# Nuralamsiddik16/Ultrafnd_git

Hardware: AMD Instinct MI355X
Metric: train-step samples/sec (FakeSV batch, seq128+224^2) (higher is better)
Workload: dtype bf16

## Files before the change

include/ultrafnd_hip.h:

```cpp
#ifndef ULTRAFND_HIP_H
#define ULTRAFND_HIP_H

#include <stddef.h>
#include <stdint.h>

#ifdef __cplusplus
extern "C" {
#endif

#define UFND_OK 0
#define UFND_ERR_INVALID 1
#define UFND_ERR_LAUNCH 2

#define UFND_ABI_VERSION 6

const char* ufnd_last_error(void);
int ufnd_abi_version(void);

typedef struct ufnd_step_state {
  uint64_t step;
  uint64_t seed;
  float lr;
  float weight_decay;
  float beta1, beta2, eps;
// ... 144 lines not shown
  float a_eps, r_eps;
  int width;
  int tile_cfg;
  const void* residual_bf16;
  int ldrb;
  float* guard;
} ufnd_gemm_ln;
#define UFND_FOLD_GUARD_SLOTS 1024
int ufnd_gemm_bf16_ln(const void* A, const void* W, const float* bias, const float* residual, void* out_bf16,
                      float* out_f32, int M, int N, int K, int lda, int ldw, int ldr, int ldo, int ldf, int act,
                      const ufnd_gemm_ln* ln, void* stream);
int ufnd_gemm_bf16_stat_parts(int M, int N, int K);

int ufnd_ln_fold_guard(const float* stats, int M, int parts, int width, float eps, float* guard, void* stream);

int ufnd_gemm_bf16_tile_count(void);
int ufnd_gemm_bf16_tile_info(int tile_cfg, int* bm, int* bn, int* ln_aware);

int ufnd_layernorm(const float* x, int ldx, const float* gamma, const float* beta, void* out_bf16, float* out_f32,
                   int M, int H, float eps, void* stream);

int ufnd_attention_bf16(const void* qkv, const int32_t* key_mask, void* ctx, int B, int L, int heads,
                        void* stream);

int ufnd_qkv_attention_bf16(const void* X, const void* Wqkv, const float* bqkv, const int32_t* key_mask, void* ctx, int B, int L,
                            int heads, int ldx, int ldw, const ufnd_gemm_ln* ln, void* stream);

int ufnd_text_pack(const int32_t* mask, int B, int L, int32_t* cu_seqlens, int32_t* row_src, void* stream);
int ufnd_text_pack_bins(const int32_t* mask, int B, int L, int32_t* cu_seqlens, int32_t* row_src, int32_t* bins, int32_t* nbins,
                        void* stream);
int ufnd_bert_embed_live(const int64_t* ids, const int32_t* row_src, const int* m_live, const float* word, const float* pos,
                         const float* type0, const float* gamma, const float* beta, void* x_bf16, float* x_f32, int capacity, int L,
                         int H, int vocab, float eps, void* stream);
int ufnd_gemm_bf16_live(const void* A, const void* W, const float* bias, const float* residual, void* out_bf16, float* out_f32,
                        int M, int N, int K, int lda, int ldw, int ldr, int ldo, int ldf, int act, int tile_cfg, const int* m_live,
                        void* stream);
int ufnd_gemm_bf16_ln_live(const void* A, const void* W, const float* bias, const float* residual, void* out_bf16, float* out_f32,
                           int M, int N, int K, int lda, int ldw, int ldr, int ldo, int ldf, int act, const ufnd_gemm_ln* ln,
                           const int* m_live, void* stream);
int ufnd_qkv_attention_bf16_packed(const void* X, const void* Wqkv, const float* bqkv, const int32_t* key_mask, const int32_t* cu_seqlens,
                                   void* ctx, int B, int L, int heads, int ldx, int ldw, const ufnd_gemm_ln* ln, void* stream);
int ufnd_qkv_attention_bf16_bins(const void* X, const void* Wqkv, const float* bqkv, const int32_t* key_mask, const int32_t* cu_seqlens,
                                 const int32_t* bins, const int32_t* nbins, void* ctx, int B, int L, int heads, int ldx, int ldw,
                                 const ufnd_gemm_ln* ln, void* stream);
int ufnd_attention_bf16_varlen_masked(const void* qkv, const int32_t* cu_seqlens, const int32_t* key_mask, void* ctx, int B, int max_len,
                                      int heads, void* stream);

int ufnd_qkv_attention_bf16_vit(const void* X, const void* Wqkv, const float* bqkv, void* ctx, int N, int T, int heads, int ldx, int ldw,
                                const ufnd_gemm_ln* ln, void* stream);
int ufnd_layernorm_live(const float* x, int ldx, const float* gamma, const float* beta, void* out_bf16, float* out_f32, int capacity,
                        int H, float eps, const int* m_live, void* stream);
int ufnd_masked_meanpool_l2_live(const float* hidden, const int32_t* mask, const int32_t* cu_seqlens, float* out, int B, int L, int H,
                                 void* stream);

int ufnd_bert_embed(const int64_t* ids, const float* word, const float* pos, const float* type0, const float* gamma,
                    const float* beta, void* x_bf16, float* x_f32, int B, int L, int H, int vocab, float eps,
                    void* stream);

int ufnd_masked_meanpool_l2(const float* hidden, const int32_t* mask, float* out, int B, int L, int H,
                            void* stream);

int ufnd_field_mean_l2(const float* parts, const int32_t* valid, float* out, int N, int M, int D, void* stream);

int ufnd_vit_patchify(const float* frames, void* patches_bf16, int N, int image, int patch, void* stream);

int ufnd_vit_assemble(const float* patch_emb, const float* cls, const float* pos, const float* gamma,
                      const float* beta, float* x_f32, void* x_bf16, float* stats, int N, int P, int H, float eps,
                      void* stream);

int ufnd_l2norm_frames(const float* e, float* out, int B, int F, int D, void* stream);

#define UFND_GATHER_MAX_ITEMS 8
typedef struct ufnd_gather_item {
  const void* src;
  void* dst;
  int row_bytes;
  int64_t src_rows;
} ufnd_gather_item;
int ufnd_gather_rows(const int64_t* idx, int B, const ufnd_gather_item* items, int n_items, void* stream);

int ufnd_temporal_weight_ld(int in_dim);
size_t ufnd_temporal_workspace_floats(int B, int in_dim, int hidden);
int ufnd_temporal_align(const float* text, const float* visual, const float* w0, const float* b0, const float* w3,
                        const float* b3, float* workspace, float* out, int B, int in_dim, int vis_dim, int hidden,
                        int out_dim, float dropout_p, const ufnd_step_state* state, void* stream);

typedef struct ufnd_tcn_layer {
  const float *w, *b;
  const float *gamma, *beta;
  float *running_mean, *running_var;
} ufnd_tcn_layer;
int ufnd_tcn_weight_ld(int in_ch, int kernel);
size_t ufnd_tcn_workspace_floats(int B, int T, int in_ch, int hid, int kernel);
int ufnd_tcn_forward(const float* text_seq, int text_dim, const float* vis_seq, int vis_dim, int B, int T,
                     const ufnd_tcn_layer* layers, int n_layers, int kernel, int hid, const float* head_w,
                     const float* head_b, int out_dim, int train, float dropout_p, float momentum, float eps,
                     const ufnd_step_state* state, float* workspace, float* out, void* stream);


int ufnd_ocr_adjacency(const int32_t* offsets, const int32_t* tokens, int N, double thresh, float* adj, int ld, void* stream);

typedef struct ufnd_gcn_params {
  const float* w1;
  const float* b1;
  const float* w2;
  const float* b2;
// ... 175 lines not shown
```

ultrafnd_git_amd/_lib.py:

```python
from __future__ import annotations

import ctypes as C
from pathlib import Path
from typing import Optional

import torch

_PKG = Path(__file__).resolve().parent
LIB_PATH = _PKG / "libultrafnd_hip.so"


class UltrafndHipError(RuntimeError):
    pass


class StepState(C.Structure):
    _fields_ = [("step", C.c_uint64), ("seed", C.c_uint64), ("lr", C.c_float), ("weight_decay", C.c_float),
                ("beta1", C.c_float), ("beta2", C.c_float), ("eps", C.c_float), ("max_norm", C.c_float),
                ("grad_scale", C.c_float), ("loss", C.c_float), ("grad_norm", C.c_float), ("clip_coef", C.c_float),
                ("bc1", C.c_float), ("bc2_sqrt", C.c_float), ("micro", C.c_uint32), ("reserved", C.c_float * 2)]


class Dims(C.Structure):
    _fields_ = [("hidden", C.c_int), ("text_dim", C.c_int), ("audio_dim", C.c_int), ("visual_dim", C.c_int),
# ... 101 lines not shown
                                             I, P, P, P, I]
    lib.ufnd_classifier_backward_ex.argtypes = [C.POINTER(Dims), C.POINTER(ClfParams), C.POINTER(ClfParams), I, I, P, P, P,
                                                I, P, P, P, I, I]
    lib.ufnd_classifier_backward_ex.restype = I
    lib.ufnd_head_factor_floats.argtypes = [C.POINTER(Dims), I]
    lib.ufnd_head_factor_floats.restype = S
    lib.ufnd_head_pack_factors.argtypes = [C.POINTER(Dims), P, P, P, P, P, I, P, P, P, P]
    lib.ufnd_head_pack_factors.restype = I
    lib.ufnd_head_linear_grads_from_factors.argtypes = [C.POINTER(Dims), C.POINTER(FusionParams), C.POINTER(ClfParams), P, S, I, I, P]
    lib.ufnd_head_linear_grads_from_factors.restype = I
    lib.ufnd_head_forward_loss.argtypes = [C.POINTER(Dims), C.POINTER(FusionParams), C.POINTER(ClfParams), C.POINTER(HeadIO), I, I, P, P]
    lib.ufnd_head_forward_loss.restype = I
    lib.ufnd_head_backward.argtypes = [C.POINTER(Dims), C.POINTER(FusionParams), C.POINTER(FusionParams), C.POINTER(ClfParams), C.POINTER(ClfParams),
                                       C.POINTER(HeadIO), I, I, P, P, P, I, I]
    lib.ufnd_head_backward.restype = I
    lib.ufnd_softmax_ce.argtypes = [P, P, I, P, P, P, P]
    lib.ufnd_softmax_ce_weighted.argtypes = [P, P, I, C.c_float, C.c_float, C.c_float, P, P, P, P]
    lib.ufnd_softmax_ce_weighted.restype = I
    lib.ufnd_grad_norm.argtypes = [P, S, P, P, P]
    lib.ufnd_adamw_step.argtypes = [P, P, P, P, S, P, P]
    lib.ufnd_step_advance.argtypes = [P, P]
    lib.ufnd_clip_adamw_step.argtypes = [P, P, P, P, S, P, P, P]
    lib.ufnd_clip_adamw_step.restype = I
    lib.ufnd_grad_accumulate.argtypes = [P, P, S, I, P, P]
    lib.ufnd_grad_accumulate.restype = I
    for name in ("ufnd_fusion_forward", "ufnd_fusion_backward", "ufnd_classifier_forward", "ufnd_classifier_backward",
                 "ufnd_softmax_ce", "ufnd_grad_norm", "ufnd_adamw_step", "ufnd_step_advance"):
        getattr(lib, name).restype = I
    _declare_encoders(lib)


def _declare_encoders(lib: C.CDLL) -> None:
    P, I, S, F = C.c_void_p, C.c_int, C.c_size_t, C.c_float
    sigs = {
        "ufnd_cast_bf16": [P, P, S, P],
        "ufnd_gemm_bf16": [P] * 6 + [I] * 9 + [P],
        "ufnd_gemm_bf16_ex": [P] * 6 + [I] * 10 + [P],
        "ufnd_layernorm": [P, I, P, P, P, P, I, I, F, P],
        "ufnd_attention_bf16": [P, P, P, I, I, I, P],
        "ufnd_qkv_attention_bf16": [P, P, P, P, P, I, I, I, I, I, C.POINTER(GemmLn), P],
        "ufnd_bert_embed": [P] * 8 + [I, I, I, I, F, P],
        "ufnd_masked_meanpool_l2": [P, P, P, I, I, I, P],
        "ufnd_text_pack": [P, I, I, P, P, P],
        "ufnd_text_pack_bins": [P, I, I, P, P, P, P, P],
        "ufnd_bert_embed_live": [P] * 10 + [I, I, I, I, F, P],
        "ufnd_gemm_bf16_live": [P] * 6 + [I] * 10 + [P, P],
        "ufnd_gemm_bf16_ln_live": [P] * 6 + [I] * 9 + [C.POINTER(GemmLn), P, P],
        "ufnd_qkv_attention_bf16_packed": [P, P, P, P, P, P, I, I, I, I, I, C.POINTER(GemmLn), P],
        "ufnd_qkv_attention_bf16_bins": [P] * 8 + [I, I, I, I, I, C.POINTER(GemmLn), P],
        "ufnd_qkv_attention_bf16_vit": [P, P, P, P, I, I, I, I, I, C.POINTER(GemmLn), P],
        "ufnd_attention_bf16_varlen_masked": [P, P, P, P, I, I, I, P],
        "ufnd_layernorm_live": [P, I, P, P, P, P, I, I, F, P, P],
        "ufnd_masked_meanpool_l2_live": [P, P, P, P, I, I, I, P],
        "ufnd_vit_patchify": [P, P, I, I, I, P],
        "ufnd_vit_assemble": [P] * 8 + [I, I, I, F, P],
        "ufnd_gemm_bf16_ln": [P] * 6 + [I] * 9 + [C.POINTER(GemmLn), P],
        "ufnd_gemm_bf16_stat_parts": [I, I, I],
        "ufnd_ln_fold_guard": [P, I, I, I, F, P, P],
        "ufnd_gemm_bf16_tile_count": [],
        "ufnd_gemm_bf16_tile_info": [I, C.POINTER(I), C.POINTER(I), C.POINTER(I)],
        "ufnd_stream_create_cu_mask": [C.POINTER(C.c_uint32), I, C.POINTER(P)],
        "ufnd_stream_destroy": [P],
        "ufnd_device_cu_count": [],
        "ufnd_l2norm_frames": [P, P, I, I, I, P],
        "ufnd_field_mean_l2": [P, P, P, I, I, I, P],
        "ufnd_temporal_align": [P] * 8 + [I] * 5 + [F, P, P],
    }
    sigs.update({
        "ufnd_gemm_bf16_dgrad": [P] * 6 + [I] * 10 + [P],
        "ufnd_gemm_bf16_wgrad": [P, P, P, I, I, I, I, I, I, P, I, P],
        "ufnd_transpose_bf16": [P, I, I, I, I, P, I, I, P, P, I, P],
        "ufnd_linear_wgrad": [P, I, P, I, I, I, I, P, P, P, P, I, P, P, C.POINTER(PartialsJob), I, P],
        "ufnd_refresh_operands": [P, I, I, P],
        "ufnd_layernorm_bwd_blocks": [I],
        "ufnd_row_partials_finish": [C.POINTER(PartialsJob), I, P],
        "ufnd_attention_bf16_lse": [P, P, P, P, I, I, I, P],
        "ufnd_attention_bf16_bwd": [P, P, P, P, P, P, P, I, I, I, P],
        "ufnd_layernorm_bwd": [P, I, P, P, I, P, I, P, P, I, P, P, P, I, I, I, F, P],
        "ufnd_masked_meanpool_l2_bwd": [P, P, P, P, I, I, I, P],
        "ufnd_l2norm_frames_bwd": [P, P, P, I, I, I, P],
        "ufnd_bert_embed_bwd": [P, P, P, P, P, I, I, I, I, I, I, P],
        "ufnd_vit_assemble_bwd": [P, P, P, P, I, I, I, P],
        "ufnd_act_bf16": [P, P, S, I, P],
        "ufnd_attention_bf16_lse_dropout": [P, P, P, P, I, I, I, C.POINTER(Dropout), P],
        "ufnd_attention_bf16_bwd_dropout": [P, P, P, P, P, P, P, I, I, I, C.POINTER(Dropout), P],
        "ufnd_dropout_residual_layernorm": [P, I, P, I, P, P, P, P, P, I, I, F, C.POINTER(Dropout), P],
        "ufnd_layernorm_dropout": [P, I, P, P, P, P, I, I, F, C.POINTER(Dropout), P],
        "ufnd_layernorm_bwd_dropout": [P, I, P, P, I, P, I, P, P, I, P, P, P, I, I, I, F, C.POINTER(Dropout), I, P],
    })
    sigs.update({
        "ufnd_wave_normalize": [P, P, P, P, I, I, P],
        "ufnd_w2v2_conv0": [P] * 8 + [I, I, I, F, P],
        "ufnd_conv1d_rows_bf16": [P] * 5 + [I] * 8 + [P],
        "ufnd_w2v2_pos_pack": [P, P, P, I, I, P],
        "ufnd_w2v2_pos_add": [P, P, P, P, I, I, P],
        "ufnd_w2v2_frames": [P, P, P, I, I, P],
        "ufnd_masked_meanpool": [P, P, P, I, I, I, P],
        "ufnd_linear_f32": [P, P, P, P, I, I, I, P],
    })
    for name, argtypes in sigs.items():
        fn = getattr(lib, name)
        fn.argtypes = argtypes
        fn.restype = I
    for name, argtypes in (("ufnd_gemm_bf16_wgrad_workspace_floats", [I, I, I]), ("ufnd_transpose_colsum_workspace_floats", [I, I]),
                           ("ufnd_attention_bwd_workspace_floats", [I, I, I]), ("ufnd_layernorm_bwd_workspace_floats", [I, I])):
        fn = getattr(lib, name)
# ... 107 lines not shown
```

ultrafnd_git_amd/csrc/encoders.hip:

```cpp
#include "common.hpp"

namespace {

__device__ __forceinline__ f32x4 ld4(const float* p) { return *reinterpret_cast<const f32x4*>(p); }

template <int NI>
__device__ __forceinline__ void ln_row(f32x4 (&v)[NI], int H, float eps, const float* gamma, const float* beta, int lane) {
  float s = 0.0f;
#pragma unroll
  for (int i = 0; i < NI; ++i) s += v[i][0] + v[i][1] + v[i][2] + v[i][3];
  const float mean = wave_sum(s) / (float)H;
  float q = 0.0f;
#pragma unroll
  for (int i = 0; i < NI; ++i)
#pragma unroll
    for (int k = 0; k < 4; ++k) {
      const float d = v[i][k] - mean;
      q += d * d;
    }
  const float rstd = rsqrtf(wave_sum(q) / (float)H + eps);
#pragma unroll
  for (int i = 0; i < NI; ++i) {
    const int col = 4 * lane + 256 * i;
    const f32x4 gm = ld4(gamma + col), bt = ld4(beta + col);
// ... 81 lines not shown
  long long id = ids[src];
  id = id < 0 ? 0 : (id >= vocab ? vocab - 1 : id);
  int l = src % L;
  l = l < 0 ? 0 : (l >= L ? L - 1 : l);
  f32x4 v[NI];
#pragma unroll
  for (int i = 0; i < NI; ++i) {
    const int col = 4 * lane + 256 * i;
    v[i] = ld4(word + (size_t)id * H + col) + ld4(pos + (size_t)l * H + col) + ld4(type0 + col);
  }
  if (gamma) ln_row<NI>(v, H, eps, gamma, beta, lane);
  store_row<NI>(v, ob, of, row, H, lane);
}

template <bool PACKED>
__global__ __launch_bounds__(256) void meanpool_kernel(const float* hidden, const int32_t* mask, float* out, int L, int H, const int32_t* cu) {
  __shared__ f32x4 part[4][64];
  __shared__ float cnts[4];
  const int b = blockIdx.y, col = blockIdx.x * 256 + 4 * (threadIdx.x & 63), grp = threadIdx.x >> 6, lane = threadIdx.x & 63;
  f32x4 acc = {0.f, 0.f, 0.f, 0.f};
  float cnt = 0.0f;
  const size_t r0 = PACKED ? (size_t)cu[b] : (size_t)b * L;
  const int n = PACKED ? cu[b + 1] - cu[b] : L;
  for (int l0 = grp; l0 < n; l0 += 32) {
    int mk[8];
    f32x4 x[8];
#pragma unroll
    for (int u = 0; u < 8; ++u) {
      const int l = l0 + 4 * u;
      mk[u] = l < n ? mask[(size_t)b * L + l] : 0;
    }
#pragma unroll
    for (int u = 0; u < 8; ++u) {
      const int l = l0 + 4 * u < n ? l0 + 4 * u : n - 1;
      x[u] = ld4(hidden + (r0 + l) * H + col);
    }
#pragma unroll
    for (int u = 0; u < 8; ++u) {
      if (mk[u] != 0) {
        acc += x[u];
        cnt += 1.0f;
      }
    }
  }
  part[grp][lane] = acc;
  if (lane == 0) cnts[grp] = cnt;
  __syncthreads();
  if (grp == 0) {
    const f32x4 s = (part[0][lane] + part[1][lane]) + (part[2][lane] + part[3][lane]);
    const float denom = fmaxf((cnts[0] + cnts[1]) + (cnts[2] + cnts[3]), 1e-6f);
    *reinterpret_cast<f32x4*>(out + (size_t)b * H + col) = s / denom;
  }
}
constexpr int PACK_THREADS = 1024, PACK_MAX_B = 16384;
__global__ __launch_bounds__(PACK_THREADS) void text_pack_kernel(const int32_t* mask, int B, int L, int32_t* cu, int32_t* row_src,
                                                                 int32_t* bins, int32_t* nbins) {
  __shared__ int lens[PACK_MAX_B];
  __shared__ int wsum[PACK_THREADS / 64];
  __shared__ long long csum[PACK_THREADS / 64];
  __shared__ int total;
  const int tid = threadIdx.x, wave = tid >> 6, lane = tid & 63;
  for (int b = wave; b < B; b += PACK_THREADS / 64) {
    int last = 0;
    for (int l = lane; l < L; l += 64) last = mask[(size_t)b * L + l] != 0 ? l + 1 : last;
#pragma unroll
    for (int o = 32; o >= 1; o >>= 1) last = max(last, __shfl_xor(last, o, 64));
    if (lane == 0) lens[b] = last;
  }
  __syncthreads();
  const int per = (B + PACK_THREADS - 1) / PACK_THREADS, b0 = tid * per, b1 = min(b0 + per, B);
  int own = 0;
  for (int b = b0; b < b1; ++b) own += lens[b];
  int inc = own;
#pragma unroll
  for (int o = 1; o < 64; o <<= 1) {
    const int y = __shfl_up(inc, o, 64);
    if (lane >= o) inc += y;
  }
  if (lane == 63) wsum[wave] = inc;
  __syncthreads();
  int base = 0;
  for (int w = 0; w < wave; ++w) base += wsum[w];
  int run = base + inc - own;
  for (int b = b0; b < b1; ++b) {
    const int n = lens[b];
    lens[b] = run;
    cu[b] = run;
    run += n;
  }
  if (tid == PACK_THREADS - 1) {
    cu[B] = run;
    total = run;
  }
  __syncthreads();
  for (int b = wave; b < B; b += PACK_THREADS / 64) {
    const int r0 = lens[b], n = (b + 1 < B ? lens[b + 1] : total) - r0;
    for (int l = lane; l < n; l += 64) row_src[r0 + l] = b * L + l;
  }
  if (!bins) return;
  auto nrows = [&](int b) { return (b + 1 < B ? lens[b + 1] : total) - lens[b]; };
  long long cown = 0;
  for (int b = b0; b < b1; ++b) {
    const int c = (nrows(b) + 31) >> 5;
    if (c > 0) cown += 1ll << (16 * (c - 1));
  }
  long long cinc = cown;
// ... 268 lines not shown
  UFND_REQUIRE(mask && cu_seqlens && row_src, "text_pack: null argument");
  UFND_REQUIRE(B >= 1 && B <= PACK_MAX_B && L >= 1 && (long long)B * L < (1ll << 31), "text_pack: B=%d L=%d (B <= %d)", B, L, PACK_MAX_B);
  hipLaunchKernelGGL(text_pack_kernel, dim3(1), dim3(PACK_THREADS), 0, (hipStream_t)stream_, mask, B, L, cu_seqlens, row_src,
                     (int32_t*)nullptr, (int32_t*)nullptr);
  UFND_CHECK_LAUNCH();
  return UFND_OK;
}

extern "C" int ufnd_text_pack_bins(const int32_t* mask, int B, int L, int32_t* cu_seqlens, int32_t* row_src, int32_t* bins,
                                   int32_t* nbins, void* stream_) {
  UFND_REQUIRE(mask && cu_seqlens && row_src && bins && nbins, "text_pack_bins: null argument");
  UFND_REQUIRE(B >= 1 && B <= PACK_MAX_B && L >= 1 && L <= 128, "text_pack_bins: B=%d L=%d (B <= %d, L <= 128)", B, L, PACK_MAX_B);
  hipLaunchKernelGGL(text_pack_kernel, dim3(1), dim3(PACK_THREADS), 0, (hipStream_t)stream_, mask, B, L, cu_seqlens, row_src, bins, nbins);
  UFND_CHECK_LAUNCH();
  return UFND_OK;
}

extern "C" int ufnd_bert_embed_live(const int64_t* ids, const int32_t* row_src, const int* m_live, const float* word, const float* pos,
                                    const float* type0, const float* gamma, const float* beta, void* x_bf16, float* x_f32, int capacity,
                                    int L, int H, int vocab, float eps, void* stream_) {
  UFND_REQUIRE(ids && row_src && m_live && word && pos && type0 && gamma && beta && (x_bf16 || x_f32), "bert_embed_live: null argument");
  UFND_REQUIRE(h_ok(H) && capacity >= 1 && L >= 1 && vocab >= 1, "bert_embed_live: capacity=%d L=%d H=%d vocab=%d", capacity, L, H, vocab);
  UFND_REQUIRE(ufnd_aligned(word, 16) && ufnd_aligned(pos, 16) && ufnd_aligned(type0, 16) &&
                   (!x_f32 || ufnd_aligned(x_f32, 16)) && (!x_bf16 || ufnd_aligned(x_bf16, 8)), "bert_embed_live: alignment");
  NI_LAUNCH(H, bert_embed_kernel, dim3(ufnd_cdiv(capacity, 4)), (hipStream_t)stream_, ids, word, pos, type0, gamma, beta,
            (__bf16*)x_bf16, x_f32, capacity, L, H, vocab, eps, row_src, m_live);
  UFND_CHECK_LAUNCH();
  return UFND_OK;
}

extern "C" int ufnd_layernorm_live(const float* x, int ldx, const float* gamma, const float* beta, void* out_bf16, float* out_f32,
                                   int capacity, int H, float eps, const int* m_live, void* stream_) {
  UFND_REQUIRE(x && gamma && beta && (out_bf16 || out_f32) && m_live && capacity >= 1, "layernorm_live: null argument");
  UFND_REQUIRE(h_ok(H), "layernorm_live: H=%d (supported 256/512/768/1024)", H);
  UFND_REQUIRE(ldx % 4 == 0 && ldx >= H && ufnd_aligned(x, 16) && ufnd_aligned(gamma, 16) && ufnd_aligned(beta, 16) &&
                   (!out_f32 || ufnd_aligned(out_f32, 16)) && (!out_bf16 || ufnd_aligned(out_bf16, 8)), "layernorm_live: alignment");
  NI_LAUNCH(H, layernorm_kernel, dim3(ufnd_cdiv(capacity, 4)), (hipStream_t)stream_, x, ldx, gamma, beta, (__bf16*)out_bf16,
            out_f32, capacity, H, eps, m_live);
  UFND_CHECK_LAUNCH();
  return UFND_OK;
}

extern "C" int ufnd_masked_meanpool_l2_live(const float* hidden, const int32_t* mask, const int32_t* cu_seqlens, float* out, int B, int L,
                                            int H, void* stream_) {
  UFND_REQUIRE(hidden && mask && cu_seqlens && out && B >= 1 && L >= 1, "meanpool_live: null argument");
  UFND_REQUIRE(H >= 256 && H % 256 == 0 && ufnd_aligned(hidden, 16) && ufnd_aligned(out, 16), "meanpool_live: H=%d (multiple of 256)", H);
  hipLaunchKernelGGL(meanpool_kernel<true>, dim3(H / 256, B), dim3(256), 0, (hipStream_t)stream_, hidden, mask, out, L, H, cu_seqlens);
  UFND_CHECK_LAUNCH();
  hipLaunchKernelGGL(l2norm_rows_kernel, dim3(B), dim3(256), 0, (hipStream_t)stream_, out, H);
  UFND_CHECK_LAUNCH();
  return UFND_OK;
}

extern "C" int ufnd_vit_patchify(const float* frames, void* patches, int N, int image, int patch, void* stream_) {
  UFND_REQUIRE(frames && patches && N >= 1, "patchify: null argument");
  UFND_REQUIRE(patch % 8 == 0 && image % patch == 0 && ufnd_aligned(frames, 16) && ufnd_aligned(patches, 16),
               "patchify: image=%d patch=%d (patch a multiple of 8, 16-B aligned buffers)", image, patch);
  const int G = image / patch;
  if (patch == 32 && G == 7) hipLaunchKernelGGL((patchify_kernel<32, 7>), dim3(N * G), dim3(256), 0, (hipStream_t)stream_, frames, (__bf16*)patches, image, patch);
  else hipLaunchKernelGGL((patchify_kernel<0, 0>), dim3(N * G), dim3(256), 0, (hipStream_t)stream_, frames, (__bf16*)patches, image, patch);
  UFND_CHECK_LAUNCH();
  return UFND_OK;
}

extern "C" int ufnd_vit_assemble(const float* patch_emb, const float* cls, const float* pos, const float* gamma,
                                 const float* beta, float* x_f32, void* x_bf16, float* stats, int N, int P, int H, float eps,
                                 void* stream_) {
  UFND_REQUIRE(patch_emb && cls && pos && ((gamma && beta) || (!gamma && !beta)) && (x_f32 || x_bf16) && N >= 1 && P >= 1, "vit_assemble: null argument");
  UFND_REQUIRE(h_ok(H), "vit_assemble: H=%d", H);
  const int M = N * (P + 1);
  UFND_REQUIRE(!stats || ufnd_aligned(stats, 16), "vit_assemble: stats alignment");
  UFND_REQUIRE((!x_f32 || ufnd_aligned(x_f32, 16)) && (!x_bf16 || ufnd_aligned(x_bf16, 8)), "vit_assemble: alignment");
  NI_LAUNCH(H, vit_assemble_kernel, dim3(ufnd_cdiv(M, 4)), (hipStream_t)stream_, patch_emb, cls, pos, gamma, beta, x_f32,
            (__bf16*)x_bf16, stats, M, P, H, eps);
  UFND_CHECK_LAUNCH();
  return UFND_OK;
}

extern "C" int ufnd_l2norm_frames(const float* e, float* out, int B, int F, int D, void* stream_) {
  UFND_REQUIRE(e && out && B >= 1 && F >= 1 && D >= 1 && D <= 1024, "l2norm_frames: B=%d F=%d D=%d", B, F, D);
  hipLaunchKernelGGL(l2norm_frames_kernel, dim3(B), dim3(256), 0, (hipStream_t)stream_, e, out, F, D);
  UFND_CHECK_LAUNCH();
  return UFND_OK;
}

extern "C" int ufnd_field_mean_l2(const float* parts, const int32_t* valid, float* out, int N, int Mx, int D, void* stream_) {
  UFND_REQUIRE(parts && valid && out && N >= 1 && Mx >= 1 && D >= 1 && D <= 1024, "field_mean_l2: N=%d M=%d D=%d", N, Mx, D);
  hipLaunchKernelGGL(field_mean_l2_kernel, dim3(N), dim3(256), 0, (hipStream_t)stream_, parts, valid, out, Mx, D);
  UFND_CHECK_LAUNCH();
  return UFND_OK;
}

namespace {
__global__ __launch_bounds__(256) void ln_fold_guard_kernel(const float* stats, int M, int parts, float inv_h, float eps, float* guard) {
  __shared__ float sh[4];
  float worst = 0.0f;
  const int nq = parts >> 1, sub = threadIdx.x & 3;
  const long long total = M;
  const long long step = (long long)gridDim.x * 64;
  for (long long r = (long long)blockIdx.x * 64 + (threadIdx.x >> 2); r < total; r += 2 * step) {
    f32x4 v[2][3];
    bool live[2];
#pragma unroll
    for (int k = 0; k < 2; ++k) {
      const long long rk = r + k * step;
      live[k] = rk < total;
// ... 47 lines not shown
```

ultrafnd_git_amd/encoders.py:

```python
from __future__ import annotations

import ctypes
import warnings
from collections import OrderedDict
from typing import Dict, NamedTuple, Optional, Tuple

import torch
import torch.nn as nn

from . import _lib as L

ACT_NONE, ACT_GELU, ACT_QUICK_GELU = 0, 1, 2


def _bf16(t: torch.Tensor) -> torch.Tensor:
    t = t.contiguous()
    out = torch.empty(t.shape, dtype=torch.bfloat16, device=t.device)
    L.check(L.lib().ufnd_cast_bf16(t.data_ptr(), out.data_ptr(), t.numel(), L.stream_ptr(t.device)), "ufnd_cast_bf16")
    return out


def dropout_prob(name: str, p) -> float:
    p = float(p)
    if not 0.0 <= p < 1.0:
# ... 255 lines not shown
                if i > 0:
                    prev = layers[-2]
                    wq = torch.cat([w[P + f"attention.self.{n}.weight"] for n in ("query", "key", "value")], 0)
                    ly["wqkvf"], ly["csqkv"], ly["bqkvf"] = self._fold(wq, ly["bqkv"], prev["g2"], prev["b2n"])
            self._packed = {"layers": layers}
        return self._packed

    def _workbufs(self, B: int, Lq: int) -> dict:
        key = (B, Lq)
        if key not in self._bufs:
            dev, M, H = self.device, B * Lq, self.hidden
            bf, f32 = dict(dtype=torch.bfloat16, device=dev), dict(dtype=torch.float32, device=dev)
            self._bufs[key] = {"xb": torch.empty(M, H, **bf), "xf": torch.empty(M, H, **f32), "y": torch.empty(M, H, **f32),
                               "x1b": torch.empty(M, H, **bf), "x1f": torch.empty(M, H, **f32),
                               "qkv": torch.empty(M, 3 * H, **bf), "ctx": torch.empty(M, H, **bf),
                               "h": torch.empty(M, self.inter, **bf), "feat": torch.empty(B, H, **f32),
                               "cu": torch.zeros(B + 1, dtype=torch.int32, device=dev), "row_src": torch.zeros(M, dtype=torch.int32, device=dev),
                               "bins": torch.zeros(B, 8, dtype=torch.int32, device=dev), "nbins": torch.zeros(1, dtype=torch.int32, device=dev)}
            p1 = self._fold_parts(M)
            if p1:
                self._bufs[key].update({"y2": torch.empty(M, H, **f32), "y1b": torch.empty(M, H, **bf), "y2b": torch.empty(M, H, **bf),
                                        "st": torch.zeros(2 * self.layers, M, p1, 2, **f32)})
                self._guard_buf(dev)
        return self._bufs[key]

    def _pass(self, input_ids: torch.Tensor, attention_mask: torch.Tensor, packed: bool, n_layers: Optional[int] = None, pool: bool = True) -> dict:
        self._require_hip()
        dev = self.device
        B, Lq = input_ids.shape
        if Lq > self.max_position:
            raise RuntimeError(f"sequence length {Lq} exceeds max_position_embeddings {self.max_position}")
        ids = input_ids.to(dev, torch.int64).contiguous()
        mask = attention_mask.to(dev, torch.int32).contiguous()
        p, b, w = self._pack(), self._workbufs(B, Lq), self._w
        M, H, s = B * Lq, self.hidden, L.stream_ptr(dev)
        t = _TextPass(B, Lq, mask, fuse=self.fuse_qkv_attention and Lq == 128 and self.heads % 2 == 0)
        if packed:
            t = t._replace(cu=b["cu"], live=b["cu"].data_ptr() + 4 * B)
            if t.fuse:
                t = t._replace(bins=b["bins"], nbins=b["nbins"])
                L.check(L.lib().ufnd_text_pack_bins(mask.data_ptr(), B, Lq, b["cu"].data_ptr(), b["row_src"].data_ptr(), b["bins"].data_ptr(),
                                                    b["nbins"].data_ptr(), s), "ufnd_text_pack_bins")
            else:
                L.check(L.lib().ufnd_text_pack(mask.data_ptr(), B, Lq, b["cu"].data_ptr(), b["row_src"].data_ptr(), s), "ufnd_text_pack")
        tables = [w["embeddings." + n].data_ptr() for n in ("word_embeddings.weight", "position_embeddings.weight", "token_type_embeddings.weight",
                                                            "LayerNorm.weight", "LayerNorm.bias")]
        outs = (b["xb"].data_ptr(), None if ("st" in b and self.residual_dtype == "bf16") else b["xf"].data_ptr())
        if packed:
            L.check(L.lib().ufnd_bert_embed_live(ids.data_ptr(), b["row_src"].data_ptr(), t.live, *tables, *outs, M, Lq, H, self.vocab, self.eps, s),
                    "ufnd_bert_embed_live")
        else:
            L.check(L.lib().ufnd_bert_embed(ids.data_ptr(), *tables, *outs, B, Lq, H, self.vocab, self.eps, s), "ufnd_bert_embed")
        layers = p["layers"] if n_layers is None else p["layers"][:max(1, int(n_layers))]
        (self._layers_folded if "st" in b else self._layers)(layers, b, t)
        if pool and packed:
            L.check(L.lib().ufnd_masked_meanpool_l2_live(b["xf"].data_ptr(), mask.data_ptr(), b["cu"].data_ptr(), b["feat"].data_ptr(), B, Lq, H, s),
                    "ufnd_masked_meanpool_l2_live")
        elif pool:
            L.check(L.lib().ufnd_masked_meanpool_l2(b["xf"].data_ptr(), mask.data_ptr(), b["feat"].data_ptr(), B, Lq, H, s), "ufnd_masked_meanpool_l2")
        return b

    def _self_attention(self, t: _TextPass, b, A, W, bias, a_stats=None, colsum=None) -> None:
        if t.fuse:
            self._qkv_attn(A, W, bias, t.mask, b["ctx"], t.B, t.Lq, self.heads, a_stats=a_stats, colsum=colsum, eps=self.eps,
                           cu=t.cu, bins=t.bins, nbins=t.nbins)
            return
        if a_stats is None:
            self._gemm(A, W, bias, out_bf16=b["qkv"], which="qkv", m_live=t.live)
        else:
            self._gemm_ln(A, W, bias, out_bf16=b["qkv"], a_stats=a_stats, colsum=colsum, eps=self.eps, which="qkv", m_live=t.live)
        if t.cu is None:
            self._attn(b["qkv"], t.mask, b["ctx"], t.B, t.Lq, self.heads)
        else:
            L.check(L.lib().ufnd_attention_bf16_varlen_masked(b["qkv"].data_ptr(), t.cu.data_ptr(), t.mask.data_ptr(), b["ctx"].data_ptr(), t.B, t.Lq,
                                                              self.heads, L.stream_ptr(self.device)), "ufnd_attention_bf16_varlen_masked")

    def _layers(self, layers, b, t: _TextPass) -> None:
        M, H, eps, live = t.B * t.Lq, self.hidden, self.eps, t.live
        for ly in layers:
            self._self_attention(t, b, b["xb"], ly["wqkv"], ly["bqkv"])
            self._gemm(b["ctx"], ly["wo"], ly["bo"], out_f32=b["y"], residual=b["xf"], which="out", m_live=live)
            self._ln(b["y"], H, ly["g1"], ly["b1"], b["x1b"], b["x1f"], M, H, eps, m_live=live)
            self._gemm(b["x1b"], ly["w1"], ly["bi"], out_bf16=b["h"], act=ACT_GELU, which="ffn1", m_live=live)
            self._gemm(b["h"], ly["w2"], ly["b2"], out_f32=b["y"], residual=b["x1f"], which="ffn2", m_live=live)
            self._ln(b["y"], H, ly["g2"], ly["b2n"], b["xb"], b["xf"], M, H, eps, m_live=live)

    def _layers_folded(self, layers, b, t: _TextPass) -> None:
        M, H, eps, live = t.B * t.Lq, self.hidden, self.eps, t.live
        y1, y2, st = b["y"], b["y2"], b["st"]
        rb = self.residual_dtype == "bf16"
        prev = None
        for i, ly in enumerate(layers):
            st1, st2 = st[2 * i], st[2 * i + 1]
            last = i == len(layers) - 1
            if prev is None:
                self._self_attention(t, b, b["xb"], ly["wqkv"], ly["bqkv"])
                self._gemm_ln(b["ctx"], ly["wo"], ly["bo"], out_f32=None if rb else y1, out_bf16=b["y1b"], residual=None if rb else b["xf"],
                              residual_bf16=b["xb"] if rb else None, out_stats=st1, eps=eps, which="out", m_live=live)
            else:
                stp = st[2 * i - 1]
                self._self_attention(t, b, b["y2b"], ly["wqkvf"], ly["bqkvf"], a_stats=stp, colsum=ly["csqkv"])
                self._gemm_ln(b["ctx"], ly["wo"], ly["bo"], out_f32=None if rb else y1, out_bf16=b["y1b"], residual=None if rb else y2,
                              residual_bf16=b["y2b"] if rb else None, r_stats=stp, r_gamma=prev["g2"], r_beta=prev["b2n"], out_stats=st1,
                              eps=eps, which="out", m_live=live)
            self._gemm_ln(b["y1b"], ly["w1f"], ly["bif"], out_bf16=b["h"], act=ACT_GELU, a_stats=st1, colsum=ly["cs1"], eps=eps, which="ffn1",
                          m_live=live)
            self._gemm_ln(b["h"], ly["w2"], ly["b2"], out_f32=y2 if (last or not rb) else None, out_bf16=b["y2b"], residual=None if rb else y1,
                          residual_bf16=b["y1b"] if rb else None, r_stats=st1, r_gamma=ly["g1"], r_beta=ly["b1"], out_stats=st2, eps=eps,
                          which="ffn2", m_live=live)
            prev = ly
        self._ln(y2, H, prev["g2"], prev["b2n"], None, b["xf"], M, H, eps, m_live=live)

    @torch.no_grad()
    def last_hidden_state(self, input_ids: torch.Tensor, attention_mask: torch.Tensor, n_layers: Optional[int] = None) -> torch.Tensor:
        b = self._pass(input_ids, attention_mask, packed=False, n_layers=n_layers, pool=False)
        return b["xf"].view(*input_ids.shape, self.hidden)

    @torch.no_grad()
    def forward(self, input_ids: torch.Tensor, attention_mask: torch.Tensor, unpad: bool = True, strict: bool = False) -> torch.Tensor:
        if strict:
            return self._strict(lambda: self.forward(input_ids, attention_mask, unpad=unpad))
        return self._pass(input_ids, attention_mask, packed=unpad)["feat"]

    encode_batch = forward

    @torch.no_grad()
    def encode_fields(self, input_ids: torch.Tensor, attention_mask: torch.Tensor, part_valid: torch.Tensor,
                      chunk: int = 1024, unpad: bool = True) -> torch.Tensor:
        self._require_hip()
        dev = self.device
        N, Mx, Lq = input_ids.shape
        valid = part_valid.to(dev, torch.int32).contiguous()
        ids = input_ids.to(dev, torch.int64).reshape(N * Mx, Lq)
        mask = attention_mask.to(dev, torch.int32).reshape(N * Mx, Lq)
        rows = torch.nonzero(valid.reshape(-1), as_tuple=False).flatten()
        parts = torch.zeros(N * Mx, self.hidden, dtype=torch.float32, device=dev)
        for s0 in range(0, rows.numel(), chunk):
            r = rows[s0:s0 + chunk]
            parts[r] = self.forward(ids[r], mask[r], unpad=unpad, strict=True)
        out = torch.empty(N, self.hidden, dtype=torch.float32, device=dev)
        L.check(L.lib().ufnd_field_mean_l2(parts.data_ptr(), valid.data_ptr(), out.data_ptr(), N, Mx, self.hidden,
                                           L.stream_ptr(dev)), "ufnd_field_mean_l2")
        return out


class ClipVisualEncoder(_EncoderBase):
    def __init__(self, layers: int = 12, hidden: int = 768, heads: int = 12, intermediate: int = 3072, patch: int = 32,
                 image: int = 224, projection_dim: int = 512, eps: float = 1e-5, fold_ln: bool = True, residual_dtype: str = "bf16",
                 attention_dropout: float = 0.0):
        super().__init__(hidden, heads, fold_ln, residual_dtype)
        self.attention_dropout = dropout_prob("attention_dropout", attention_dropout)
        self.layers, self.inter = layers, intermediate
        self.patch, self.image, self.proj, self.eps = patch, image, projection_dim, eps
        self.n_patches = (image // patch) ** 2
        self.fuse_qkv_attention = True
        w, V, init = self._w, "vision_model.", self._seeded_init()
        w[V + "embeddings.class_embedding"] = init((hidden,))
        w[V + "embeddings.patch_embedding.weight"] = init((hidden, 3, patch, patch))
        w[V + "embeddings.position_embedding.weight"] = init((self.n_patches + 1, hidden))
        w[V + "pre_layrnorm.weight"], w[V + "pre_layrnorm.bias"] = torch.ones(hidden), torch.zeros(hidden)
        for i in range(layers):
            P = V + f"encoder.layers.{i}."
            for n in ("k_proj", "v_proj", "q_proj", "out_proj"):
                w[P + f"self_attn.{n}.weight"] = init((hidden, hidden))
                w[P + f"self_attn.{n}.bias"] = torch.zeros(hidden)
            w[P + "layer_norm1.weight"], w[P + "layer_norm1.bias"] = torch.ones(hidden), torch.zeros(hidden)
            w[P + "mlp.fc1.weight"], w[P + "mlp.fc1.bias"] = init((intermediate, hidden)), torch.zeros(intermediate)
            w[P + "mlp.fc2.weight"], w[P + "mlp.fc2.bias"] = init((hidden, intermediate)), torch.zeros(hidden)
            w[P + "layer_norm2.weight"], w[P + "layer_norm2.bias"] = torch.ones(hidden), torch.zeros(hidden)
        w[V + "post_layernorm.weight"], w[V + "post_layernorm.bias"] = torch.ones(hidden), torch.zeros(hidden)
        w["visual_projection.weight"] = init((projection_dim, hidden))

    def _pack(self):
        if self._packed is None:
            w, V, layers = self._w, "vision_model.", []
            for i in range(self.layers):
                P = V + f"encoder.layers.{i}."
                layers.append({
                    "wqkv": _bf16(torch.cat([w[P + f"self_attn.{n}.weight"] for n in ("q_proj", "k_proj", "v_proj")], 0)),
                    "bqkv": torch.cat([w[P + f"self_attn.{n}.bias"] for n in ("q_proj", "k_proj", "v_proj")], 0).contiguous(),
                    "wo": _bf16(w[P + "self_attn.out_proj.weight"]), "bo": w[P + "self_attn.out_proj.bias"],
                    "g1": w[P + "layer_norm1.weight"], "b1": w[P + "layer_norm1.bias"],
                    "w1": _bf16(w[P + "mlp.fc1.weight"]), "bi": w[P + "mlp.fc1.bias"],
                    "w2": _bf16(w[P + "mlp.fc2.weight"]), "b2": w[P + "mlp.fc2.bias"],
                    "g2": w[P + "layer_norm2.weight"], "b2n": w[P + "layer_norm2.bias"]})
                ly = layers[-1]
                wq = torch.cat([w[P + f"self_attn.{n}.weight"] for n in ("q_proj", "k_proj", "v_proj")], 0)
                ly["wqkvf"], ly["csqkv"], ly["bqkvf"] = self._fold(wq, ly["bqkv"], ly["g1"], ly["b1"])
                ly["w1f"], ly["cs1"], ly["bif"] = self._fold(w[P + "mlp.fc1.weight"], ly["bi"], ly["g2"], ly["b2n"])
            self._packed = {"layers": layers,
                            "wpatch": _bf16(w[V + "embeddings.patch_embedding.weight"].reshape(self.hidden, -1)),
                            "wproj": _bf16(w["visual_projection.weight"])}
        return self._packed

    def _workbufs(self, B: int, Fr: int) -> dict:
        key = (B, Fr)
        if key not in self._bufs:
            dev, H, N = self.device, self.hidden, B * Fr
            T = self.n_patches + 1
            M = N * T
            bf, f32 = dict(dtype=torch.bfloat16, device=dev), dict(dtype=torch.float32, device=dev)
            self._bufs[key] = {"patches": torch.empty(N * self.n_patches, 3 * self.patch ** 2, **bf),
                               "pe": torch.empty(N * self.n_patches, H, **f32), "xf": torch.empty(M, H, **f32),
                               "hb": torch.empty(M, H, **bf), "qkv": torch.empty(M, 3 * H, **bf),
                               "ctx": torch.empty(M, H, **bf), "m": torch.empty(M, self.inter, **bf),
                               "pooled": torch.empty(N, H, **bf), "e": torch.empty(N, self.proj, **f32),
                               "feat": torch.empty(B, self.proj, **f32)}
            p1 = self._fold_parts(M)
            if p1:
                self._bufs[key].update({"st0": torch.zeros(M, 2, 2, **f32), "st": torch.zeros(2 * self.layers, M, p1, 2, **f32)})
                self._guard_buf(dev)
        return self._bufs[key]

    @torch.no_grad()
    def image_embeds(self, frames: torch.Tensor) -> torch.Tensor:
        return self._run(frames[:, None])[0]

    @torch.no_grad()
    def hidden_state(self, frames: torch.Tensor, n_layers: Optional[int] = None) -> torch.Tensor:
        if frames.dim() == 4:
            frames = frames[:, None]
        _, b = self._run(frames, n_layers)
        N = frames.shape[0] * frames.shape[1]
        return b["xf"].view(N, self.n_patches + 1, self.hidden)

    def _embed(self, fr, p, b, N) -> None:
        w, V, s = self._w, "vision_model.", L.stream_ptr(self.device)
        L.check(L.lib().ufnd_vit_patchify(fr.data_ptr(), b["patches"].data_ptr(), N, self.image, self.patch, s), "ufnd_vit_patchify")
        self._gemm(b["patches"], p["wpatch"], None, out_f32=b["pe"])
        L.check(L.lib().ufnd_vit_assemble(b["pe"].data_ptr(), w[V + "embeddings.class_embedding"].data_ptr(),
                                          w[V + "embeddings.position_embedding.weight"].data_ptr(),
                                          w[V + "pre_layrnorm.weight"].data_ptr(), w[V + "pre_layrnorm.bias"].data_ptr(),
                                          None if ("st0" in b and self.residual_dtype == "bf16") else b["xf"].data_ptr(),
                                          L.ptr(b["hb"]) if "st0" in b else None, L.ptr(b.get("st0")),
                                          N, self.n_patches, self.hidden, self.eps, s), "ufnd_vit_assemble")

    def _blocks_folded(self, layers, b, N) -> None:
        eps, stA, st, T = self.eps, b["st0"], b["st"], self.n_patches + 1
        rb = self.residual_dtype == "bf16"
        fuse = self.fuse_qkv_attention and T <= 64
        for i, ly in enumerate(layers):
            st1, st2 = st[2 * i], st[2 * i + 1]
            last = i == len(layers) - 1
            if fuse:
                self._qkv_attn(b["hb"], ly["wqkvf"], ly["bqkvf"], None, b["ctx"], N, T, self.heads, a_stats=stA, colsum=ly["csqkv"], eps=eps)
            else:
                self._gemm_ln(b["hb"], ly["wqkvf"], ly["bqkvf"], out_bf16=b["qkv"], a_stats=stA, colsum=ly["csqkv"], eps=eps, which="qkv")
                self._attn(b["qkv"], None, b["ctx"], N, T, self.heads)
            self._gemm_ln(b["ctx"], ly["wo"], ly["bo"], out_f32=None if rb else b["xf"], out_bf16=b["hb"], residual=None if rb else b["xf"],
                          residual_bf16=b["hb"] if rb else None, out_stats=st1, eps=eps, which="out")
            self._gemm_ln(b["hb"], ly["w1f"], ly["bif"], out_bf16=b["m"], act=ACT_QUICK_GELU, a_stats=st1, colsum=ly["cs1"], eps=eps, which="ffn1")
            self._gemm_ln(b["m"], ly["w2"], ly["b2"], out_f32=b["xf"] if (last or not rb) else None, out_bf16=b["hb"],
                          residual=None if rb else b["xf"], residual_bf16=b["hb"] if rb else None, out_stats=st2, eps=eps, which="ffn2")
            stA = st2

    def _blocks(self, layers, b, N) -> None:
        H, T, eps = self.hidden, self.n_patches + 1, self.eps
        M = N * T
        fuse = self.fuse_qkv_attention and T <= 64
        for ly in layers:
            self._ln(b["xf"], H, ly["g1"], ly["b1"], b["hb"], None, M, H, eps)
            if fuse:
                self._qkv_attn(b["hb"], ly["wqkv"], ly["bqkv"], None, b["ctx"], N, T, self.heads)
            else:
                self._gemm(b["hb"], ly["wqkv"], ly["bqkv"], out_bf16=b["qkv"], which="qkv")
                self._attn(b["qkv"], None, b["ctx"], N, T, self.heads)
            self._gemm(b["ctx"], ly["wo"], ly["bo"], out_f32=b["xf"], residual=b["xf"], which="out")
            self._ln(b["xf"], H, ly["g2"], ly["b2n"], b["hb"], None, M, H, eps)
            self._gemm(b["hb"], ly["w1"], ly["bi"], out_bf16=b["m"], act=ACT_QUICK_GELU, which="ffn1")
            self._gemm(b["m"], ly["w2"], ly["b2"], out_f32=b["xf"], residual=b["xf"], which="ffn2")

    def _pooled_projection(self, p, b, N) -> None:
        w, V, H = self._w, "vision_model.", self.hidden
        self._ln(b["xf"], (self.n_patches + 1) * H, w[V + "post_layernorm.weight"], w[V + "post_layernorm.bias"], b["pooled"], None, N, H, self.eps)
        self._gemm(b["pooled"], p["wproj"], None, out_f32=b["e"])

    def _run(self, frames5: torch.Tensor, n_layers: Optional[int] = None):
        self._require_hip()
        B, Fr = frames5.shape[:2]
        if tuple(frames5.shape[2:]) != (3, self.image, self.image):
            raise RuntimeError(f"frames: expected (B,F,3,{self.image},{self.image}), got {tuple(frames5.shape)}")
        fr = L.f32c(frames5.to(self.device)).view(B * Fr, 3, self.image, self.image)
        p, b = self._pack(), self._workbufs(B, Fr)
        layers = p["layers"] if n_layers is None else p["layers"][:max(1, int(n_layers))]
        self._embed(fr, p, b, B * Fr)
        (self._blocks_folded if "st0" in b else self._blocks)(layers, b, B * Fr)
        self._pooled_projection(p, b, B * Fr)
        return b["e"], b

    @torch.no_grad()
    def forward(self, frames: torch.Tensor, strict: bool = False) -> torch.Tensor:
        if frames.dim() == 4:
            frames = frames[:, None]
        if strict:
            return self._strict(lambda: self.forward(frames))
        B, Fr = frames.shape[:2]
        e, b = self._run(frames)
        L.check(L.lib().ufnd_l2norm_frames(e.data_ptr(), b["feat"].data_ptr(), B, Fr, self.proj, L.stream_ptr(self.device)),
                "ufnd_l2norm_frames")
        return b["feat"]
```

Before: 28690.

## Fuse text final LayerNorm into meanpool and compute ViT last layer on CLS rows

Two changes. On the text side, the last LayerNorm of the folded BERT path is fused into the masked mean-pool kernel, which normalizes each row while pooling, so the separate full-sequence LN pass and its fp32 write-back are skipped. On the vision side, the last transformer block runs the out-projection, FFN1 and FFN2 only on the CLS token rows, because only the CLS output feeds the pooled projection; this cuts the tail GEMMs by a factor of the token count. The cost is extra strided views, new stat buffers, and a new kernel that recomputes LN per row, and the full last hidden state is no longer materialized.

```diff
diff --git a/include/ultrafnd_hip.h b/include/ultrafnd_hip.h
--- a/include/ultrafnd_hip.h
+++ b/include/ultrafnd_hip.h
@@ -220,6 +220,8 @@
                         int H, float eps, const int* m_live, void* stream);
 int ufnd_masked_meanpool_l2_live(const float* hidden, const int32_t* mask, const int32_t* cu_seqlens, float* out, int B, int L, int H,
                                  void* stream);
+int ufnd_ln_masked_meanpool_l2_live(const float* y, const float* gamma, const float* beta, float eps, const int32_t* mask,
+                                    const int32_t* cu_seqlens, float* out, int B, int L, int H, void* stream);
 
 int ufnd_bert_embed(const int64_t* ids, const float* word, const float* pos, const float* type0, const float* gamma,
                     const float* beta, void* x_bf16, float* x_f32, int B, int L, int H, int vocab, float eps,
diff --git a/ultrafnd_git_amd/_lib.py b/ultrafnd_git_amd/_lib.py
--- a/ultrafnd_git_amd/_lib.py
+++ b/ultrafnd_git_amd/_lib.py
@@ -177,6 +177,7 @@
         "ufnd_attention_bf16_varlen_masked": [P, P, P, P, I, I, I, P],
         "ufnd_layernorm_live": [P, I, P, P, P, P, I, I, F, P, P],
         "ufnd_masked_meanpool_l2_live": [P, P, P, P, I, I, I, P],
+        "ufnd_ln_masked_meanpool_l2_live": [P, P, P, F, P, P, P, I, I, I, P],
         "ufnd_vit_patchify": [P, P, I, I, I, P],
         "ufnd_vit_assemble": [P] * 8 + [I, I, I, F, P],
         "ufnd_gemm_bf16_ln": [P] * 6 + [I] * 9 + [C.POINTER(GemmLn), P],
diff --git a/ultrafnd_git_amd/csrc/encoders.hip b/ultrafnd_git_amd/csrc/encoders.hip
--- a/ultrafnd_git_amd/csrc/encoders.hip
+++ b/ultrafnd_git_amd/csrc/encoders.hip
@@ -157,6 +157,57 @@
     *reinterpret_cast<f32x4*>(out + (size_t)b * H + col) = s / denom;
   }
 }
+template <int NI>
+__global__ __launch_bounds__(256) void ln_meanpool_kernel(const float* y, const float* gamma, const float* beta, float eps, const int32_t* mask,
+                                                          const int32_t* cu, float* out, int L, int H) {
+  __shared__ f32x4 part[4][NI][64];
+  __shared__ float cnts[4];
+  const int b = blockIdx.x, grp = __builtin_amdgcn_readfirstlane(threadIdx.x >> 6), lane = threadIdx.x & 63;
+  const size_t r0 = (size_t)cu[b];
+  const int n = cu[b + 1] - cu[b];
+  f32x4 acc[NI];
+#pragma unroll
+  for (int i = 0; i < NI; ++i) acc[i] = f32x4{0.f, 0.f, 0.f, 0.f};
+  float cnt = 0.0f;
+  for (int l0 = grp; l0 < n; l0 += 32) {
+    int mk[8];
+    f32x4 v[8][NI];
+#pragma unroll
+    for (int u = 0; u < 8; ++u) {
+      const int l = l0 + 4 * u;
+      mk[u] = l < n ? mask[(size_t)b * L + l] : 0;
+    }
+#pragma unroll
+    for (int u = 0; u < 8; ++u) {
+      const int l = l0 + 4 * u < n ? l0 + 4 * u : n - 1;
+#pragma unroll
+      for (int i = 0; i < NI; ++i) v[u][i] = ld4(y + (r0 + l) * H + 4 * lane + 256 * i);
+    }
+#pragma unroll
+    for (int u = 0; u < 8; ++u) ln_row<NI>(v[u], H, eps, gamma, beta, lane);
+#pragma unroll
+    for (int u = 0; u < 8; ++u) {
+      if (mk[u] != 0) {
+#pragma unroll
+        for (int i = 0; i < NI; ++i) acc[i] += v[u][i];
+        cnt += 1.0f;
+      }
+    }
+  }
+#pragma unroll
+  for (int i = 0; i < NI; ++i) part[grp][i][lane] = acc[i];
+  if (lane == 0) cnts[grp] = cnt;
+  __syncthreads();
+  if (grp == 0) {
+    const float denom = fmaxf((cnts[0] + cnts[1]) + (cnts[2] + cnts[3]), 1e-6f);
+#pragma unroll
+    for (int i = 0; i < NI; ++i) {
+      const f32x4 s = (part[0][i][lane] + part[1][i][lane]) + (part[2][i][lane] + part[3][i][lane]);
+      *reinterpret_cast<f32x4*>(out + (size_t)b * H + 4 * lane + 256 * i) = s / denom;
+    }
+  }
+}
+
 constexpr int PACK_THREADS = 1024, PACK_MAX_B = 16384;
 __global__ __launch_bounds__(PACK_THREADS) void text_pack_kernel(const int32_t* mask, int B, int L, int32_t* cu, int32_t* row_src,
                                                                  int32_t* bins, int32_t* nbins) {
@@ -531,6 +582,18 @@
   return UFND_OK;
 }
 
+extern "C" int ufnd_ln_masked_meanpool_l2_live(const float* y, const float* gamma, const float* beta, float eps, const int32_t* mask,
+                                               const int32_t* cu_seqlens, float* out, int B, int L, int H, void* stream_) {
+  UFND_REQUIRE(y && gamma && beta && mask && cu_seqlens && out && B >= 1 && L >= 1, "ln_meanpool_live: null argument");
+  UFND_REQUIRE(h_ok(H), "ln_meanpool_live: H=%d (supported 256/512/768/1024)", H);
+  UFND_REQUIRE(ufnd_aligned(y, 16) && ufnd_aligned(gamma, 16) && ufnd_aligned(beta, 16) && ufnd_aligned(out, 16), "ln_meanpool_live: alignment");
+  NI_LAUNCH(H, ln_meanpool_kernel, dim3(B), (hipStream_t)stream_, y, gamma, beta, eps, mask, cu_seqlens, out, L, H);
+  UFND_CHECK_LAUNCH();
+  hipLaunchKernelGGL(l2norm_rows_kernel, dim3(B), dim3(256), 0, (hipStream_t)stream_, out, H);
+  UFND_CHECK_LAUNCH();
+  return UFND_OK;
+}
+
 extern "C" int ufnd_vit_patchify(const float* frames, void* patches, int N, int image, int patch, void* stream_) {
   UFND_REQUIRE(frames && patches && N >= 1, "patchify: null argument");
   UFND_REQUIRE(patch % 8 == 0 && image % patch == 0 && ufnd_aligned(frames, 16) && ufnd_aligned(patches, 16),
diff --git a/ultrafnd_git_amd/encoders.py b/ultrafnd_git_amd/encoders.py
--- a/ultrafnd_git_amd/encoders.py
+++ b/ultrafnd_git_amd/encoders.py
@@ -331,8 +331,16 @@
         else:
             L.check(L.lib().ufnd_bert_embed(ids.data_ptr(), *tables, *outs, B, Lq, H, self.vocab, self.eps, s), "ufnd_bert_embed")
         layers = p["layers"] if n_layers is None else p["layers"][:max(1, int(n_layers))]
-        (self._layers_folded if "st" in b else self._layers)(layers, b, t)
-        if pool and packed:
+        ln_pool = pool and packed and "st" in b
+        if "st" in b:
+            self._layers_folded(layers, b, t, final_ln=not ln_pool)
+        else:
+            self._layers(layers, b, t)
+        if ln_pool:
+            L.check(L.lib().ufnd_ln_masked_meanpool_l2_live(b["y2"].data_ptr(), layers[-1]["g2"].data_ptr(), layers[-1]["b2n"].data_ptr(), self.eps,
+                                                            mask.data_ptr(), b["cu"].data_ptr(), b["feat"].data_ptr(), B, Lq, H, s),
+                    "ufnd_ln_masked_meanpool_l2_live")
+        elif pool and packed:
             L.check(L.lib().ufnd_masked_meanpool_l2_live(b["xf"].data_ptr(), mask.data_ptr(), b["cu"].data_ptr(), b["feat"].data_ptr(), B, Lq, H, s),
                     "ufnd_masked_meanpool_l2_live")
         elif pool:
@@ -364,7 +372,7 @@
             self._gemm(b["h"], ly["w2"], ly["b2"], out_f32=b["y"], residual=b["x1f"], which="ffn2", m_live=live)
             self._ln(b["y"], H, ly["g2"], ly["b2n"], b["xb"], b["xf"], M, H, eps, m_live=live)
 
-    def _layers_folded(self, layers, b, t: _TextPass) -> None:
+    def _layers_folded(self, layers, b, t: _TextPass, final_ln: bool = True) -> None:
         M, H, eps, live = t.B * t.Lq, self.hidden, self.eps, t.live
         y1, y2, st = b["y"], b["y2"], b["st"]
         rb = self.residual_dtype == "bf16"
@@ -388,7 +396,8 @@
                           residual_bf16=b["y1b"] if rb else None, r_stats=st1, r_gamma=ly["g1"], r_beta=ly["b1"], out_stats=st2, eps=eps,
                           which="ffn2", m_live=live)
             prev = ly
-        self._ln(y2, H, prev["g2"], prev["b2n"], None, b["xf"], M, H, eps, m_live=live)
+        if final_ln:
+            self._ln(y2, H, prev["g2"], prev["b2n"], None, b["xf"], M, H, eps, m_live=live)
 
     @torch.no_grad()
     def last_hidden_state(self, input_ids: torch.Tensor, attention_mask: torch.Tensor, n_layers: Optional[int] = None) -> torch.Tensor:
@@ -433,6 +442,7 @@
         self.patch, self.image, self.proj, self.eps = patch, image, projection_dim, eps
         self.n_patches = (image // patch) ** 2
         self.fuse_qkv_attention = True
+        self.cls_tail = True
         w, V, init = self._w, "vision_model.", self._seeded_init()
         w[V + "embeddings.class_embedding"] = init((hidden,))
         w[V + "embeddings.patch_embedding.weight"] = init((hidden, 3, patch, patch))
@@ -487,13 +497,16 @@
                                "feat": torch.empty(B, self.proj, **f32)}
             p1 = self._fold_parts(M)
             if p1:
-                self._bufs[key].update({"st0": torch.zeros(M, 2, 2, **f32), "st": torch.zeros(2 * self.layers, M, p1, 2, **f32)})
+                self._bufs[key].update({"st0": torch.zeros(M, 2, 2, **f32), "st": torch.zeros(2 * self.layers, M, p1, 2, **f32),
+                                        "stc": torch.zeros(2, N, p1, 2, **f32)})
                 self._guard_buf(dev)
+            else:
+                self._bufs[key]["hc"] = torch.empty(N, H, **bf)
         return self._bufs[key]
 
     @torch.no_grad()
     def image_embeds(self, frames: torch.Tensor) -> torch.Tensor:
-        return self._run(frames[:, None])[0]
+        return self._run(frames[:, None], cls_tail=self.cls_tail)[0]
 
     @torch.no_grad()
     def hidden_state(self, frames: torch.Tensor, n_layers: Optional[int] = None) -> torch.Tensor:
@@ -514,7 +527,17 @@
                                           L.ptr(b["hb"]) if "st0" in b else None, L.ptr(b.get("st0")),
                                           N, self.n_patches, self.hidden, self.eps, s), "ufnd_vit_assemble")
 
-    def _blocks_folded(self, layers, b, N) -> None:
+    def _cls_rows(self, b, N) -> dict:
+        T = self.n_patches + 1
+        r = {k: b[k].view(N, T * self.hidden)[:, :self.hidden] for k in ("ctx", "hb", "xf")}
+        r["m"] = b["m"][:N]
+        if "stc" in b:
+            r["st1"], r["st2"] = b["stc"][0], b["stc"][1]
+        else:
+            r["hb"] = b["hc"]
+        return r
+
+    def _blocks_folded(self, layers, b, N, cls_tail: bool = False) -> None:
         eps, stA, st, T = self.eps, b["st0"], b["st"], self.n_patches + 1
         rb = self.residual_dtype == "bf16"
         fuse = self.fuse_qkv_attention and T <= 64
@@ -526,35 +549,41 @@
             else:
                 self._gemm_ln(b["hb"], ly["wqkvf"], ly["bqkvf"], out_bf16=b["qkv"], a_stats=stA, colsum=ly["csqkv"], eps=eps, which="qkv")
                 self._attn(b["qkv"], None, b["ctx"], N, T, self.heads)
-            self._gemm_ln(b["ctx"], ly["wo"], ly["bo"], out_f32=None if rb else b["xf"], out_bf16=b["hb"], residual=None if rb else b["xf"],
-                          residual_bf16=b["hb"] if rb else None, out_stats=st1, eps=eps, which="out")
-            self._gemm_ln(b["hb"], ly["w1f"], ly["bif"], out_bf16=b["m"], act=ACT_QUICK_GELU, a_stats=st1, colsum=ly["cs1"], eps=eps, which="ffn1")
-            self._gemm_ln(b["m"], ly["w2"], ly["b2"], out_f32=b["xf"] if (last or not rb) else None, out_bf16=b["hb"],
-                          residual=None if rb else b["xf"], residual_bf16=b["hb"] if rb else None, out_stats=st2, eps=eps, which="ffn2")
+            r = b
+            if last and cls_tail:
+                r = self._cls_rows(b, N)
+                st1, st2 = r["st1"], r["st2"]
+            self._gemm_ln(r["ctx"], ly["wo"], ly["bo"], out_f32=None if rb else r["xf"], out_bf16=r["hb"], residual=None if rb else r["xf"],
+                          residual_bf16=r["hb"] if rb else None, out_stats=st1, eps=eps, which="out")
+            self._gemm_ln(r["hb"], ly["w1f"], ly["bif"], out_bf16=r["m"], act=ACT_QUICK_GELU, a_stats=st1, colsum=ly["cs1"], eps=eps, which="ffn1")
+            self._gemm_ln(r["m"], ly["w2"], ly["b2"], out_f32=r["xf"] if (last or not rb) else None, out_bf16=r["hb"],
+                          residual=None if rb else r["xf"], residual_bf16=r["hb"] if rb else None, out_stats=st2, eps=eps, which="ffn2")
             stA = st2
 
-    def _blocks(self, layers, b, N) -> None:
+    def _blocks(self, layers, b, N, cls_tail: bool = False) -> None:
         H, T, eps = self.hidden, self.n_patches + 1, self.eps
         M = N * T
         fuse = self.fuse_qkv_attention and T <= 64
-        for ly in layers:
+        for i, ly in enumerate(layers):
             self._ln(b["xf"], H, ly["g1"], ly["b1"], b["hb"], None, M, H, eps)
             if fuse:
                 self._qkv_attn(b["hb"], ly["wqkv"], ly["bqkv"], None, b["ctx"], N, T, self.heads)
             else:
                 self._gemm(b["hb"], ly["wqkv"], ly["bqkv"], out_bf16=b["qkv"], which="qkv")
                 self._attn(b["qkv"], None, b["ctx"], N, T, self.heads)
-            self._gemm(b["ctx"], ly["wo"], ly["bo"], out_f32=b["xf"], residual=b["xf"], which="out")
-            self._ln(b["xf"], H, ly["g2"], ly["b2n"], b["hb"], None, M, H, eps)
-            self._gemm(b["hb"], ly["w1"], ly["bi"], out_bf16=b["m"], act=ACT_QUICK_GELU, which="ffn1")
-            self._gemm(b["m"], ly["w2"], ly["b2"], out_f32=b["xf"], residual=b["xf"], which="ffn2")
+            r = self._cls_rows(b, N) if (cls_tail and i == len(layers) - 1) else b
+            xf = r["xf"]
+            self._gemm(r["ctx"], ly["wo"], ly["bo"], out_f32=xf, residual=xf, which="out")
+            self._ln(xf, xf.stride(0), ly["g2"], ly["b2n"], r["hb"], None, xf.shape[0], H, eps)
+            self._gemm(r["hb"], ly["w1"], ly["bi"], out_bf16=r["m"], act=ACT_QUICK_GELU, which="ffn1")
+            self._gemm(r["m"], ly["w2"], ly["b2"], out_f32=xf, residual=xf, which="ffn2")
 
     def _pooled_projection(self, p, b, N) -> None:
         w, V, H = self._w, "vision_model.", self.hidden
         self._ln(b["xf"], (self.n_patches + 1) * H, w[V + "post_layernorm.weight"], w[V + "post_layernorm.bias"], b["pooled"], None, N, H, self.eps)
         self._gemm(b["pooled"], p["wproj"], None, out_f32=b["e"])
 
-    def _run(self, frames5: torch.Tensor, n_layers: Optional[int] = None):
+    def _run(self, frames5: torch.Tensor, n_layers: Optional[int] = None, cls_tail: bool = False):
         self._require_hip()
         B, Fr = frames5.shape[:2]
         if tuple(frames5.shape[2:]) != (3, self.image, self.image):
@@ -563,7 +592,7 @@
         p, b = self._pack(), self._workbufs(B, Fr)
         layers = p["layers"] if n_layers is None else p["layers"][:max(1, int(n_layers))]
         self._embed(fr, p, b, B * Fr)
-        (self._blocks_folded if "st0" in b else self._blocks)(layers, b, B * Fr)
+        (self._blocks_folded if "st0" in b else self._blocks)(layers, b, B * Fr, cls_tail)
         self._pooled_projection(p, b, B * Fr)
         return b["e"], b
 
@@ -574,7 +603,7 @@
         if strict:
             return self._strict(lambda: self.forward(frames))
         B, Fr = frames.shape[:2]
-        e, b = self._run(frames)
+        e, b = self._run(frames, cls_tail=self.cls_tail)
         L.check(L.lib().ufnd_l2norm_frames(e.data_ptr(), b["feat"].data_ptr(), B, Fr, self.proj, L.stream_ptr(self.device)),
                 "ufnd_l2norm_frames")
         return b["feat"]
```

Result: faster. 29120, median of 6 (+1.5%).
